# LaurenYTaylor/jsrl-CORL

Hardware: AMD Instinct MI355X
Metric: IQL gradient-steps/sec at batch=256 (D4RL obs/act dims) (higher is better)
Workload: dtype f32; 1 GPU; IQL step on synthetic buffer (obs=17, act=6, 1000000 rows), batch=256 per GPU; global_batch=256, parallelism=single, prepare_rehearsal_steps=1111

## Files before the change

jsrl-corl_amd/csrc/iqlhip.hip:

```cpp
#include "iqlhip_kernels.h"
#include "iqlhip_lb_kernels.h"
#include "iqlhip_owned.h"

#include <dlfcn.h>

#include <time.h>

#include <algorithm>
#include <cstdarg>
#include <cstdio>
#include <cstdlib>
#include <cstring>
#include <memory>
#include <string>
#include <type_traits>
#include <vector>

#define GRAPH_STEPS IQLHIP_GRAPH_STEPS
static const int kChunkSizes[] = {GRAPH_STEPS, 16, 4, 2, 1};

static thread_local std::string g_err;

static int fail(int code, const char* fmt, ...) {
  char buf[512];
// ... 21 lines not shown
  static err_t dev_fill(void* p, int byte, size_t n) { return hipMemset(p, byte, n); }
  static err_t dev_free(void* p) { return hipFree(p); }
  static err_t pin_alloc(void** p, size_t n) { return hipHostMalloc(p, n, hipHostMallocDefault); }
  static err_t pin_free(void* p) { return hipHostFree(p); }
  static err_t event_create(event_t* e, unsigned flags) { return hipEventCreateWithFlags(e, flags); }
  static err_t event_destroy(event_t e) { return hipEventDestroy(e); }
};
using Owned = OwnedT<HipApi>;
extern "C" int64_t iqlhip_debug_live_buffers(void) { return Owned::live().load(std::memory_order_relaxed); }
template <class F> static int all_or_nothing(Owned& own, F&& allocate) {
  const size_t mark = own.mark();
  const int rc = allocate();
  if (rc) own.rollback(mark);
  return rc;
}

template <class F> static auto with_bools(F&& f) { return f(); }
template <class F, class... Bs> static auto with_bools(F&& f, bool b, Bs... rest) {
  if (!b) return with_bools([&](auto... t) { return f(std::false_type{}, t...); }, rest...);
  return with_bools([&](auto... t) { return f(std::true_type{}, t...); }, rest...);
}
static auto fwd_one_kernel(bool bf, bool dma) {
  return with_bools([](auto BF, auto DMA) { return &iql_fwd_kernel<BF.value, DMA.value, false, true>; }, bf, dma);
}
static auto fwd_kernel(bool bf, bool dma, bool multi) {
  return with_bools([](auto MU, auto BF, auto DMA) { return &iql_fwd_kernel<BF.value, DMA.value, MU.value>; }, multi, bf, dma);
}
static auto bwd_kernel(bool bf, bool full, bool multi) {
  return with_bools([](auto MU, auto BF, auto FU) { return &iql_bwd_kernel<BF.value, FU.value, MU.value>; }, multi, bf, full);
}
using BwdRwFn = void (*)(const float*, const float*, const float*, const float*, const float*, unsigned, unsigned, unsigned,
                         unsigned, StepParams, const float*, float*);
static BwdRwFn bwd_rw_kernel(bool full, bool multi);
static auto bwd_rows_kernel(bool csplit) {
  return with_bools([](auto CS) { return &iql_bwd_rows_kernel<CS.value>; }, csplit);
}
template <class Sel> static int set_max_lds(int n_flags, size_t lds, Sel sel) {
  for (unsigned m = 0; m < (1u << n_flags); ++m)
    HIPCHK(hipFuncSetAttribute((const void*)sel(m), hipFuncAttributeMaxDynamicSharedMemorySize, (int)lds));
  return IQLHIP_OK;
}

static inline double now_us() {
  timespec ts;
  clock_gettime(CLOCK_MONOTONIC, &ts);
  return ts.tv_sec * 1e6 + ts.tv_nsec * 1e-3;
}
static const bool g_trace = getenv("IQLHIP_TRACE") != nullptr;

static int check_host_indices(const int64_t* idx_host, int64_t n, int64_t n_rows) {
  for (int64_t i = 0; i < n; ++i)
    if (idx_host[i] < 0 || idx_host[i] >= n_rows)
      return fail(IQLHIP_EINDEX, "index %lld is out of bounds for dimension 0 with size %lld", (long long)idx_host[i], (long long)n_rows);
  return IQLHIP_OK;
}

struct DevGuard {
  int prev = -1;
  bool switched = false;
  explicit DevGuard(int dev) {
    if (hipGetDevice(&prev) == hipSuccess && prev != dev) switched = (hipSetDevice(dev) == hipSuccess);
  }
  ~DevGuard() { if (switched) (void)hipSetDevice(prev); }
};

struct PrioSrc { unsigned* stamp = nullptr; unsigned* flags = nullptr; unsigned long long* delta = nullptr; int sh0 = 0;
// ... 72 lines not shown
  unsigned long long act_drop_seed = 0, act_drop_calls = 0;
  int precision = 0;
  __bf16* wsh = nullptr;
  __bf16* tsh = nullptr;
  float* loss_ring = nullptr;
  int ring_cap = 0;
  iqlhip_step_scalars* sched_cur = nullptr;
  iqlhip_step_scalars* sched_call = nullptr;
  iqlhip_step_scalars* sched_pin[4] = {nullptr, nullptr, nullptr, nullptr};
  unsigned long long* sched_ack = nullptr;
  unsigned long long sched_want[4] = {0, 0, 0, 0};
  unsigned long long call_seq = 0;
  unsigned* setup_arrivals = nullptr;
  bool fwd_lds_set[N_CHUNK_KINDS] = {false, false, false, false, false};
  float* is_buf = nullptr;
  char* prio_buf = nullptr;
  char* prep_save = nullptr;
  hipStream_t sched_stream[4] = {nullptr, nullptr, nullptr, nullptr};
  int sched_slot = 0;
  unsigned long long* hdr = nullptr;
  unsigned long long* stamps = nullptr;
  int k_max = 0;
  int n_chunk_max = 0, n_rt_max = 0;
  size_t lds_fwd = 0, lds_fwd_solo = 0, lds_bwd = 0;
  int n_cus = 256;
  int w0_lds_k = 0;
  int bwd_donate_pct = -1;
  int bwd_spb_force = -1;
  int fwd_spb_force = -1;
  float* pi_t = nullptr;
  __bf16* dh1g = nullptr;
  float* slab_x = nullptr;
  __bf16* wimg = nullptr;
  int lb_enabled = 1;
  int lb_nbb_force = -1, lb_cpb_force = -1, lb_nbi_force = -1;
  bool lb_pi_spread = true;
  bool lb_csplit = true;
  int lb_bwd_part = 0;
  size_t lds_bwd_lb = 0;
  hipStream_t cap_stream = nullptr;
  struct CachedGraph { GraphKey key; hipGraph_t graph; hipGraphExec_t exec; unsigned long long stamp; hipStream_t last;
                       IdleWork* work;
                       hipGraphNode_t setup_node;  };
  struct { bool valid = false; const float* rows = nullptr; int64_t ld = 0, size = 0; int32_t B = 0; uint64_t seed = 0;
           uint64_t next_offset = 0; float drop_p = 0.f; uint64_t drop_seed = 0, drop_step = 0;
           uint64_t wt_gen = 0;
           int cont_class = 0;
           uint64_t wt_ver = 0;
           const void* owner = nullptr;
         } cont;
  std::vector<CachedGraph> graphs;
  unsigned long long graph_clock = 0;
  int xch_mode = IQLHIP_XCH_NONE;
  int rank = 0, world = 1;
  float* xflat = nullptr;
  void* nccl_comm = nullptr;
  char* xblk = nullptr;
  size_t xblk_bytes = 0, xflat_off[2] = {0, 0};
  size_t xslabb_off[2] = {0, 0}, xloss_off[2] = {0, 0};
  long long xslab_b_off[4] = {0, 0, 0, 0};
  char* peer_blk[IQLHIP_MAX_WORLD] = {nullptr, nullptr, nullptr, nullptr, nullptr, nullptr, nullptr, nullptr};
  bool p2p_attached = false;
  unsigned long long* xstatus = nullptr;
  unsigned long long* xstatus_host = nullptr;
  unsigned long long xstep = 0;
  unsigned long long xtimeout_ticks = 500000000ull;
// ... 112 lines not shown
    sb += (size_t)c->n_rt_max * ((size_t)HID * c->L.net[n].k_in + HID);
  }
  HIPCHK(dalloc(&c->sc.slab_b, sb));
  HIPCHK(dalloc(&c->sc.loss_parts, 2 * 4 * 64));
  HIPCHK(dalloc(&c->pi_t, (size_t)MB * 65));
  HIPCHK(dalloc(&c->sc.losses, 4));
  HIPCHK(dalloc(&c->flat_tmp, (size_t)c->L.n_params + 4));
  c->k_max = 1024;
  c->ring_cap = c->k_max;
  HIPCHK(own.pin(&c->loss_ring, (size_t)c->ring_cap * 4 * sizeof(float), true));
  HIPCHK(own.dev(&c->sched_cur, (size_t)GRAPH_STEPS * sizeof(iqlhip_step_scalars)));
  HIPCHK(own.dev(&c->sched_call, (size_t)c->k_max * sizeof(iqlhip_step_scalars)));
  for (int i = 0; i < 4; ++i) HIPCHK(own.pin(&c->sched_pin[i], (size_t)c->k_max * sizeof(iqlhip_step_scalars)));
  HIPCHK(own.pin(&c->sched_ack, 8 * sizeof(unsigned long long), true));
  HIPCHK(own.dev(&c->setup_arrivals, 64, 0));
  HIPCHK(own.dev(&c->hdr, HDR_WORDS * sizeof(unsigned long long), 0));
  HIPCHK(own.dev(&c->xstatus, 2 * sizeof(unsigned long long), 0));
  HIPCHK(own.pin(&c->xstatus_host, 2 * sizeof(unsigned long long), true));
  HIPCHK(dalloc(&c->xflat, (size_t)up(c->L.n_params + 4, 64)));
  HIPCHK(hipStreamCreateWithFlags(&c->cap_stream, hipStreamNonBlocking));
#ifdef IQL_STAMPS
  HIPCHK(own.dev(&c->stamps, 4096 * 16 * sizeof(unsigned long long), 0));
#endif
  const int kq = dims->state_dim + dims->action_dim;
  const int ks_ = dims->state_dim;
  const size_t fwd_fixed = (size_t)(RT_ROWS * H0_LD + RT_ROWS * T64_LD + RT_ROWS * (int)c->row_ld +
                                    (((A + 15) & ~15) * W2_LD + 32) + 512 + 16) * sizeof(float);
  auto fits = [&](int k) { return fwd_fixed + (size_t)HID * k * sizeof(float) + 4096 <= (size_t)160 * 1024 - 1024; };
  int w0_lds_k = 0;
  if (kq <= W0_DMA_MAX_K && fits(kq)) w0_lds_k = kq;
  else if (ks_ <= W0_DMA_MAX_K && fits(ks_)) w0_lds_k = ks_;
  if (const char* ov = getenv("IQLHIP_W0_LDS_K")) w0_lds_k = std::min(w0_lds_k, atoi(ov));
  c->w0_lds_k = w0_lds_k;
  if (const char* ov = getenv("IQLHIP_BWD_DONATE_PCT")) c->bwd_donate_pct = std::max(0, std::min(100, atoi(ov)));
  if (const char* ov = getenv("IQLHIP_BWD_SPB_L2")) c->bwd_spb_force = std::max(0, std::min(2, atoi(ov)));
  if (const char* ov = getenv("IQLHIP_FWD_SPB_L2")) c->fwd_spb_force = std::max(0, std::min(2, atoi(ov)));
  if (const char* ov = getenv("IQLHIP_LB")) c->lb_enabled = atoi(ov) != 0;
  if (const char* ov = getenv("IQLHIP_LB_NBB")) c->lb_nbb_force = std::max(2, atoi(ov));
  if (const char* ov = getenv("IQLHIP_LB_CSPLIT")) c->lb_csplit = atoi(ov) != 0;
  if (const char* ov = getenv("IQLHIP_LB_PI_SPREAD")) c->lb_pi_spread = atoi(ov) != 0;
  if (const char* ov = getenv("IQLHIP_LB_CPB")) c->lb_cpb_force = std::max(1, atoi(ov));
  if (const char* ov = getenv("IQLHIP_LB_NBI")) c->lb_nbi_force = std::max(2, atoi(ov));
  c->lds_fwd = fwd_fixed + (size_t)HID * w0_lds_k * sizeof(float) + (w0_lds_k > W0_LDS_MAX_K ? 4096 : 0);
  c->lds_fwd_solo = std::max(c->lds_fwd, (size_t)(81 * 1024));
  {
    int ncu = 0;
    if (hipDeviceGetAttribute(&ncu, hipDeviceAttributeMultiprocessorCount, c->device) == hipSuccess && ncu > 0) c->n_cus = ncu;
  }
  const int dyld = ((A + 15) & ~15) + 4;
  const size_t lds_a = (size_t)(4 * 32 * T64_LD + 2 * CHUNK_ROWS * dyld + 32 * 32 + 64 + CHUNK_ROWS) * sizeof(float);
  const size_t lds_b = (size_t)(RT_ROWS * H0_LD + 4 * 32 * T64_LD + RT_ROWS * T64_LD + RT_ROWS * 36 + 4 +
                                RT_ROWS * XR_LD_MAX) * sizeof(float);
  c->lds_bwd = std::max(lds_a, lds_b);
  c->lds_bwd_lb = (size_t)(3 * 32 * H0B_LD + 32 * LB_DYLD) * 2 + 32 * 4 + (size_t)(2 * 4 * 32 + 16) * 4;
  int rc = set_max_lds(3, c->lds_fwd_solo, [](unsigned m) { return fwd_kernel(m & 1, m & 2, m & 4); });
  if (!rc) rc = set_max_lds(2, c->lds_fwd_solo, [](unsigned m) { return fwd_one_kernel(m & 1, m & 2); });
  if (!rc) rc = set_max_lds(3, c->lds_bwd, [](unsigned m) { return bwd_kernel(m & 1, m & 2, m & 4); });
  if (!rc) rc = set_max_lds(1, c->lds_bwd_lb, [](unsigned m) { return bwd_rows_kernel(m & 1); });
  if (!rc) rc = set_max_lds(2, c->lds_bwd, [](unsigned m) { return bwd_rw_kernel(m & 1, m & 2); });
  c->fwd_lds_set[(int)ChunkKind::Plain] = !rc;
  return rc;
}

extern "C" int iqlhip_create(const iqlhip_dims* dims, const iqlhip_hyper* hyper, int device, iqlhip_ctx** out) {
  int rc = check_dims(dims);
  if (rc) return rc;
  if (!hyper || !out) return fail(IQLHIP_EINVAL, "hyper/out is NULL");
  int ndev = 0;
  HIPCHK(hipGetDeviceCount(&ndev));
  if (device < 0 || device >= ndev) return fail(IQLHIP_EHIP, "device %d not available (%d visible)", device, ndev);
  DevGuard guard(device);
  iqlhip_ctx* c = new iqlhip_ctx();
  rc = create_impl(c, dims, hyper, device);
  if (rc) {
    const std::string msg = g_err;
    iqlhip_destroy(c);
    g_err = msg;
    return rc;
  }
  *out = c;
  return IQLHIP_OK;
}

static void free_graph(iqlhip_ctx::CachedGraph& g) {
  if (g.exec) (void)hipGraphExecDestroy(g.exec);
  if (g.graph) (void)hipGraphDestroy(g.graph);
  if (g.work) (void)hipFree(g.work);
}
static void drop_graph(iqlhip_ctx* c) {
  for (auto& g : c->graphs) {
    if (g.last) (void)hipStreamSynchronize(g.last);
    free_graph(g);
// ... 296 lines not shown
  u.n_loss = u.n_chunk;
  u.slab_x = nullptr;
  u.n_x = 0;
  if (use_lb(c, rows)) {
    const LbGeom gm = lb_geom(c, rows);
    u.n_chunk = gm.n_cg;
    u.slab_x = c->slab_x;
    u.n_x = gm.nbb;
    u.loss_parts = c->sc.loss_parts + 256;
    u.n_loss = 1;
  }
  u.batch_rows = rows;
  u.sched = nullptr;
  u.sched_idx = 0;
  u.ring_hdr = nullptr;
  u.adv_hdr = nullptr; u.adv_k = 0; u.adv_rows = 0;
  u.done_flag = nullptr; u.done_val = 0;
  u.wsh = (c->precision == 1) ? c->wsh : nullptr;
  u.tsh = (c->precision == 1) ? c->tsh : nullptr;
  u.wimg = (c->precision == 1 && use_lb(c, rows)) ? c->wimg : nullptr;
  if (getenv("IQLHIP_LB_NOIMG")) u.wimg = nullptr;
  u.n_peer = 0;
  u.peer_direct = 0;
  for (int r = 0; r < IQLHIP_MAX_WORLD; ++r) { u.peer_flat[r] = nullptr; u.peer_slab_b[r] = nullptr; u.peer_loss[r] = nullptr; }
  return u;
}

static size_t fwd_lds(const iqlhip_ctx* c, int n_blocks) { return (n_blocks <= c->n_cus) ? c->lds_fwd_solo : c->lds_fwd; }

static const void* fwd_kernel_of(ChunkKind kind, bool bf, bool dma, bool multi);
static void launch_fwd_grid(const iqlhip_ctx* c, const StepParams& p, int nb, hipStream_t st, ChunkKind kind = ChunkKind::Plain) {
  const bool dma = c->w0_lds_k > W0_LDS_MAX_K;
  const bool bf = c->precision == 1, multi = (p.spb_l2 & 3) > 0;
  const void* kernel = (p.only_inst >= 0) ? (const void*)fwd_one_kernel(bf, dma) : fwd_kernel_of(kind, bf, dma, multi);
  void* args[] = {const_cast<StepParams*>(&p)};
  (void)hipLaunchKernel(kernel, dim3(nb), dim3(256), args, fwd_lds(c, nb), st);
}
static int ensure_fwd_lds(iqlhip_ctx* c, ChunkKind kind) {
  if (c->fwd_lds_set[(int)kind]) return IQLHIP_OK;
  DevGuard guard(c->device);
  if (int rc = set_max_lds(3, c->lds_fwd_solo, [kind](unsigned m) { return fwd_kernel_of(kind, m & 1, m & 2, m & 4); })) return rc;
  c->fwd_lds_set[(int)kind] = true;
  return IQLHIP_OK;
}

static int fwd_spb_l2(const iqlhip_ctx* c, int n_rt) {
  if (c->fwd_spb_force >= 0) return c->fwd_spb_force;
  if (8 * n_rt * NSPLIT <= c->n_cus) return 0;
  if (8 * n_rt * 2 <= c->n_cus) return 1;
  return 2;
}
static int fwd_blocks(int n_rt, int l2) { return (l2 == 2) ? 8 * 2 * ((n_rt + 1) / 2) : 8 * n_rt * (NSPLIT >> l2); }
static void launch_fwd(const iqlhip_ctx* c, const StepParams& p_in, hipStream_t st, ChunkKind kind = ChunkKind::Plain) {
  StepParams p = p_in;
  if (p.only_inst < 0 && use_lb(c, p.rows)) {
    const LbArgs a = lb_args(c, p.rows);
    const int kq = c->dims.state_dim + c->dims.action_dim;
    const dim3 grid(8 * a.nbi);
    const bool spread = a.n_rt > 2 * a.nbi && c->lb_pi_spread;
    if (spread) {
      if (kq <= 32) hipLaunchKernelGGL((iql_fwd_lb_kernel<1, true>), grid, dim3(256), 0, st, p, a);
      else if (kq <= 64) hipLaunchKernelGGL((iql_fwd_lb_kernel<2, true>), grid, dim3(256), 0, st, p, a);
      else hipLaunchKernelGGL((iql_fwd_lb_kernel<3, true>), grid, dim3(256), 0, st, p, a);
    } else {
      if (kq <= 32) hipLaunchKernelGGL((iql_fwd_lb_kernel<1, false>), grid, dim3(256), 0, st, p, a);
      else if (kq <= 64) hipLaunchKernelGGL((iql_fwd_lb_kernel<2, false>), grid, dim3(256), 0, st, p, a);
      else hipLaunchKernelGGL((iql_fwd_lb_kernel<3, false>), grid, dim3(256), 0, st, p, a);
// ... 3737 lines not shown
                                        float alpha, float eps, void* stream) {
  if (!t || (m > 0 && (!idx_dev || !td_dev))) return fail(IQLHIP_EINVAL, "NULL argument");
  if (!t->local) return fail(IQLHIP_EINVAL, "the table is not updatable (iqlhip_weights_build_updatable)");
  if (m < 0) return fail(IQLHIP_EINVAL, "m = %lld entries", (long long)m);
  if (bound < 0 || bound > t->n) return fail(IQLHIP_EINVAL, "bound = %lld outside [0, %lld]", (long long)bound, (long long)t->n);
  if ((((uintptr_t)idx_dev) & 7) || (((uintptr_t)td_dev) & 7)) return fail(IQLHIP_EINVAL, "indices and TD errors must be 8-byte aligned");
  if (int rc = prio_exponents_check(alpha, eps)) return rc;
  DevGuard guard(t->device);
  hipStream_t st = (hipStream_t)stream;
  const WUpd u{t->tab, t->stamp, t->flags, (unsigned)t->n, t->levels, t->sh0, t->sat_bits};
  const PrioArgs a{nullptr, alpha, eps};
  for (int64_t j0 = 0; j0 < m; j0 += WT_UPDATE_SLICE) {
    const unsigned k = (unsigned)std::min<int64_t>(WT_UPDATE_SLICE, m - j0);
    launch_update_td(u, (const long long*)idx_dev + j0, td_dev + 2 * j0, k, (long long)bound, t->delta, a, st, t->q_max);
  }
  HIPCHK(hipGetLastError());
  ++t->version;
  return IQLHIP_OK;
}

static auto fwd_prio_kernel(bool dma, bool multi) {
  return with_bools([](auto MU, auto DMA) { return &iql_fwd_prio_kernel<DMA.value, MU.value>; }, multi, dma);
}
static const void* fwd_kernel_of(ChunkKind kind, bool bf, bool dma, bool multi) {
  switch (kind) {
    case ChunkKind::Plain: return (const void*)fwd_kernel(bf, dma, multi);
    case ChunkKind::Mixed: return (const void*)fwd_mixed_kernel(bf, dma, multi);
    case ChunkKind::Weighted: return (const void*)fwd_weighted_kernel(bf, dma, multi);
    case ChunkKind::WeightedIs: return (const void*)fwd_weighted_is_kernel(dma, multi);
    case ChunkKind::Prio: return (const void*)fwd_prio_kernel(dma, multi);
  }
  return nullptr;
}
static void launch_prio_update(const iqlhip_ctx* c, const ChunkSrc& src, int B, int k, hipStream_t st) {
  const WUpd u{const_cast<unsigned long long*>(src.wt.tab), src.up.stamp, src.up.flags, src.wt.n, (int)src.wt.levels, src.up.sh0,
               src.up.sat_bits};
  const PrioArgs a{prio_words(c), 0.f, 0.f};
  launch_update_td(u, prio_idx(c, k & 1), prio_td(c), (unsigned)B, (long long)src.wt.n, src.up.delta, a, st, src.up.q_max);
}
static int prio_setup(iqlhip_ctx* c, const iqlhip_weights* table, int32_t B, float alpha, float eps) {
  if (!table->local) return fail(IQLHIP_EINVAL, "the table is not updatable (iqlhip_weights_build_updatable)");
  if (int rc = prio_exponents_check(alpha, eps)) return rc;
  if (B > WT_UPDATE_SLICE) return fail(IQLHIP_EUNSUPPORTED, "prioritised calls take batches of at most %d rows", WT_UPDATE_SLICE);
  DevGuard guard(c->device);
  if (!c->prio_buf) HIPCHK(c->own.dev(&c->prio_buf, 24 * (size_t)c->dims.max_batch + 4 * sizeof(float), 0));
  return ensure_fwd_lds(c, ChunkKind::Prio);
}
static ChunkCall prio_call(const iqlhip_weights* t, float is_beta, float alpha, float eps, unsigned live) {
  ChunkCall call = weighted_call(t, ChunkKind::Prio, is_beta);
  call.src.up = PrioSrc{t->stamp, t->flags, t->delta, t->sh0, t->sat_bits, t->q_max};
  call.alpha = alpha; call.eps = eps; call.live = live;
  return call;
}
extern "C" int iqlhip_train_steps_prioritized_prepare(iqlhip_ctx* c, const float* rows_dev, int64_t ld, int32_t B,
                                                      float inv_batch, void* stream, iqlhip_weights* table) {
  int rc = check_weighted_args(c, rows_dev, ld, table ? table->n : 0, B, table);
  if (!rc) rc = weighted_is_setup(c, 0.f);
  if (!rc) rc = prio_setup(c, table, B, 1.f, 1.f);
  if (rc) return rc;
  return train_steps_prepare(c, rows_dev, ld, B, inv_batch, stream, prio_call(table, 0.f, 1.f, 1.f, 0u));
}
extern "C" int iqlhip_train_steps_prioritized(iqlhip_ctx* c, const float* rows_dev, int64_t ld, int64_t size, int32_t B,
                                              const iqlhip_step_scalars* sc, int32_t K, uint64_t seed, uint64_t stream_offset,
                                              int32_t flags, void* stream, iqlhip_weights* table, float is_beta, float alpha,
                                              float eps) {
  if (!sc) return fail(IQLHIP_EINVAL, "NULL argument");
// ... 644 lines not shown
```

jsrl-corl_amd/csrc/iqlhip_fwd_body.inc:

```
  RT_ENTRY();
  const int bid = blockIdx.x;
  const int fx = bid & 7, fh = fx >> 2, fr = bid >> 3;
  constexpr unsigned FWD_PAIR_A = 0x6541u, FWD_PAIR_B = 0x7320u;
  const int inst = ONE ? p.only_inst : (int)((((fr & 1) ? FWD_PAIR_B : FWD_PAIR_A) >> (4 * (fx & 3))) & 7u);
  if (inst >= 7) {
    if (p.g_work) idle_block_work<MIXED_IDLE>(p.g_work, (fr >> 1) * 2 + fh, (int)(gridDim.x >> 3));
    return;
  }
  const int spb_l2 = MULTI ? (p.spb_l2 & 3) : 0;
  const int spb = 1 << spb_l2;
  int ns, rt;
  if (ONE) {
    ns = bid & (NSPLIT - 1);
    rt = bid >> 2;
  } else if (spb_l2 == 0) {
    ns = 2 * ((fr >> 1) & 1) + fh;
    rt = fr >> 2;
    if (ROW_EXIT && rt * RT_ROWS >= p.rows) return;
  } else if (spb_l2 == 1) {
    ns = 2 * fh;
    rt = fr >> 1;
    if (ROW_EXIT && rt * RT_ROWS >= p.rows) return;
  } else {
    ns = 0;
    rt = 2 * (fr >> 1) + fh;
    if (rt * RT_ROWS >= p.rows) return;
  }
  const int row0 = rt * RT_ROWS;
  const int tid = threadIdx.x, lane = tid & 63, wave = tid >> 6;
  const int l15 = lane & 15, g = lane >> 4;

  const NetPtrs np = p.inst[inst];
  const int xoff = p.xoff[inst];
  const int slot = p.slot[inst];
  const int k0 = np.k0;
  const int k0p = (k0 + 3) & ~3;
  const int D = np.d;
  const int ld = p.ld;
  const int B = p.rows;
  const int w0k = p.w0_lds_k;
  const float* xb = p.xb;
  float* h0g = p.sc.h0;
  float* h1g = p.sc.h1;
  float* headsg = p.sc.heads;
  const int MB = p.sc.max_batch;
  const int Aact = p.A;
  PIN_P(np.w0); PIN_P(np.b0); PIN_P(np.w1); PIN_P(np.b1); PIN_P(np.w2); PIN_P(np.b2);
  PIN_S(k0); PIN_S(D); PIN_S(xoff); PIN_S(slot); PIN_S(ld); PIN_S(B); PIN_S(MB); PIN_S(Aact);
  PIN_P(xb); PIN_P(h0g); PIN_P(h1g); PIN_P(headsg); PIN_S(w0k);
  const bool w0_lds = W0DMA ? (k0 <= w0k) : (k0 <= min(w0k, W0_LDS_MAX_K));
  const bool w0_dma = W0DMA && w0_lds && (k0 > W0_LDS_MAX_K);

  extern __shared__ __attribute__((aligned(16))) float smem[];
  float* H0s = smem;
  float* H1s = H0s + RT_ROWS * H0_LD;
  float* Xr = H1s + RT_ROWS * T64_LD;
  float* W2s = Xr + RT_ROWS * ld;
  const int w2s_words = ((Aact + 15) & ~15) * W2_LD + 32;
  unsigned* Mk = (unsigned*)(W2s + w2s_words);
  float* W0s = W2s + w2s_words + 512;

  STAMP_BASE(p, 0);
  STAMP(p, 0);
  const int n_x = RT_ROWS * ld / 4;
  const int x_last = B * ld / 4 - 1;
  f32x4 xr[XR_MAX_F4];
  xr_load(xr, xb, row0 * ld / 4, n_x, x_last);
  f32x4 w2pre[2];
#pragma unroll
  for (int q = 0; q < 2; ++q) {
    const int e = min(tid + 256 * q, D * 16 - 1);
    w2pre[q] = *(const f32x4*)(np.w2 + (unsigned)((e >> 4) * HID + ns * 64 + 4 * (e & 15)));
  }
  const float b2v = np.b2[min(tid, D - 1)];
  f32x4 bias0[4];
#pragma unroll
  for (int ct = 0; ct < 4; ++ct) bias0[ct] = *(const f32x4*)(np.b0 + (unsigned)(wave * 64 + ct * 16 + 4 * g));
  f32x4 bias1 = *(const f32x4*)(np.b1 + (unsigned)(ns * 64 + wave * 16 + 4 * g));
  const bool drop = (inst == 6) && (p.drop_bits != nullptr);
  unsigned mk0 = 0xFFFFFFFFu, mk1 = 0xFFFFFFFFu;
  if (drop) {
    const int mrow = min(row0 + (tid >> 3), B - 1);
    mk0 = p.drop_bits[mrow * 8 + (tid & 7)];
    mk1 = p.drop_bits[(MB + mrow) * 8 + (tid & 7)];
  }
  const int n_w0v = 64 * k0;
  f32x4 w0v[16];
  if (w0_dma) {
    const int nj = (n_w0v + 255) >> 8;
    for (int j = 0; j < nj; ++j)
      lds_dma16(np.w0 + 4 * min(tid + 256 * j, n_w0v - 1), W0s + 4 * (256 * j + 64 * wave));
  } else if (w0_lds) {
#pragma unroll
    for (int j = 0; j < 8; ++j) w0v[j] = *(const f32x4*)(np.w0 + 4u * (unsigned)min(tid + 256 * j, n_w0v - 1));
    if (k0 > 32) {
#pragma unroll
      for (int j = 8; j < 16; ++j) w0v[j] = *(const f32x4*)(np.w0 + 4u * (unsigned)min(tid + 256 * j, n_w0v - 1));
    }
  }
  int n1 = ns * 64 + wave * 16 + l15;
  f32x4 bw[BF16 ? 1 : 16];
  bf16x8 bwb[BF16 ? 8 : 1];
  __bf16* H0b = (__bf16*)H0s;

  xr_store(xr, Xr, n_x);
  const int Dp = (D + 15) & ~15;
#pragma unroll
  for (int q = 0; q < 2; ++q) {
    const int e = tid + 256 * q;
    if (e < Dp * 16) *(f32x4*)(W2s + (e >> 4) * W2_LD + 4 * (e & 15)) = (e < D * 16) ? w2pre[q] : (f32x4){0.f, 0.f, 0.f, 0.f};
  }
  if (tid < D) W2s[Dp * W2_LD + tid] = b2v;
  Mk[tid] = mk0;
  Mk[256 + tid] = mk1;
  if (w0_lds && !w0_dma) {
#pragma unroll
    for (int j = 0; j < 8; ++j) {
      const int f = tid + 256 * j;
      if (f < n_w0v) *(f32x4*)(W0s + 4 * f) = w0v[j];
    }
    if (k0 > 32) {
#pragma unroll
      for (int j = 8; j < 16; ++j) {
        const int f = tid + 256 * j;
        if (f < n_w0v) *(f32x4*)(W0s + 4 * f) = w0v[j];
      }
    }
  }
  __syncthreads();
  const bool bw_in_l0 = !BF16 && w0_lds;
#define BW_LOAD(ks_) bw[ks_] = *(const f32x4*)(np.w1 + (unsigned)(n1 * HID + 16 * (ks_) + 4 * g))
#define BWB_AT(unit_, j_) (*(const bf16x8*)((const __bf16*)np.w1 + (unsigned)((unit_) * HID + 32 * (j_) + 8 * g)))
  if constexpr (BF16) {
#pragma unroll
    for (int j = 0; j < 8; ++j) bwb[j] = BWB_AT(n1, j);
  } else if (!bw_in_l0) {
#pragma unroll
    for (int ks = 0; ks < 16; ++ks) BW_LOAD(ks);
  }
  STAMP(p, 1);

  {
    f32x4 acc[2][4];
#pragma unroll
    for (int i = 0; i < 2; ++i)
#pragma unroll
      for (int j = 0; j < 4; ++j) acc[i][j] = (f32x4){0.f, 0.f, 0.f, 0.f};
    const int nks = k0p >> 2;
    const float* x0 = Xr + l15 * ld + xoff;
    const float* x1 = Xr + (16 + l15) * ld + xoff;
    float bcur[4], bnxt[4], acur[2], anxt[2];
    if (w0_lds && nks <= 8) {
      const float* wl[4];
#pragma unroll
      for (int ct = 0; ct < 4; ++ct) wl[ct] = W0s + (wave * 64 + ct * 16 + l15) * k0;
      float bq[8][4], aq[8][2];
#pragma unroll
      for (int ks = 0; ks < 8; ++ks) {
        const int kk = 4 * ks + g;
        const int kc = min(kk, k0 - 1);
#pragma unroll
        for (int ct = 0; ct < 4; ++ct) bq[ks][ct] = wl[ct][kc];
        const float xa = x0[kc], xb_ = x1[kc];
        aq[ks][0] = (kk < k0) ? xa : 0.f;
        aq[ks][1] = (kk < k0) ? xb_ : 0.f;
      }
#pragma unroll
      for (int ks = 0; ks < 8; ++ks) {
        asm volatile("" : "+v"(aq[ks][0]), "+v"(aq[ks][1]));
      }
      STAMP(p, 5);
      if constexpr (BF16) {
        l0_chunk_bf16(acc, bq, aq);
      } else {
// ... 92 lines not shown
          acc[0][ct] = MFMA16(bcur[ct], a0, acc[0][ct]);
          acc[1][ct] = MFMA16(bcur[ct], a1, acc[1][ct]);
        }
#pragma unroll
        for (int ct = 0; ct < 4; ++ct) bcur[ct] = bnxt[ct];
      }
    }
#pragma unroll
    for (int ct = 0; ct < 4; ++ct) {
#pragma unroll
      for (int rtile = 0; rtile < 2; ++rtile) {
        f32x4 h;
#pragma unroll
        for (int reg = 0; reg < 4; ++reg) h[reg] = fmaxf(acc[rtile][ct][reg] + bias0[ct][reg], 0.f);
        if (drop) {
          const unsigned bits = Mk[(rtile * 16 + l15) * 8 + wave * 2 + (ct >> 1)] >> ((ct & 1) * 16 + 4 * g);
#pragma unroll
          for (int reg = 0; reg < 4; ++reg) h[reg] = ((bits >> reg) & 1u) ? h[reg] * p.drop_scale : 0.f;
        }
        if constexpr (BF16) {
          bf16x4 hb_;
#pragma unroll
          for (int reg = 0; reg < 4; ++reg) hb_[reg] = (__bf16)h[reg];
          *(bf16x4*)(H0b + (rtile * 16 + l15) * H0B_LD + wave * 64 + ct * 16 + 4 * g) = hb_;
        } else {
          *(f32x4*)(H0s + (rtile * 16 + l15) * H0_LD + wave * 64 + ct * 16 + 4 * g) = h;
        }
      }
    }
  }
  STAMP(p, 7);
  __syncthreads();
  STAMP(p, 2);

  for (int it = 0;; ++it) {
  const bool more = MULTI && (it + 1 < spb);
  f32x4 bias1n = bias1;
  if (more) {
#pragma unroll
    for (int q = 0; q < 2; ++q) {
      const int e = min(tid + 256 * q, D * 16 - 1);
      w2pre[q] = *(const f32x4*)(np.w2 + (unsigned)((e >> 4) * HID + (ns + 1) * 64 + 4 * (e & 15)));
    }
    bias1n = *(const f32x4*)(np.b1 + (unsigned)((ns + 1) * 64 + wave * 16 + 4 * g));
  }
  if (slot >= 0) {
    const int rl = tid >> 3;
    const int row = row0 + rl;
    if (row < B) {
#pragma unroll
      for (int j = 0; j < 2; ++j) {
        const int col = ns * 64 + 4 * ((tid & 7) + 8 * j);
        if constexpr (BF16)
          *(bf16x4*)((__bf16*)h0g + (unsigned)((slot * MB + row) * HID + col)) = *(const bf16x4*)(H0b + rl * H0B_LD + col);
        else
          *(f32x4*)(h0g + (unsigned)((slot * MB + row) * HID + col)) = *(const f32x4*)(H0s + rl * H0_LD + col);
      }
    }
  }

  if (it == 0) STAMP(p, 8);
  {
    f32x4 acc0 = (f32x4){0.f, 0.f, 0.f, 0.f}, acc1 = acc0;
    if constexpr (BF16) {
      bf16x8 b0[8], b1[8];
#pragma unroll
      for (int j = 0; j < 8; ++j) {
        b0[j] = *(const bf16x8*)(H0b + l15 * H0B_LD + 32 * j + 8 * g);
        b1[j] = *(const bf16x8*)(H0b + (16 + l15) * H0B_LD + 32 * j + 8 * g);
      }
#pragma unroll
      for (int j = 0; j < 8; ++j) {
        acc0 = MFMA_BF16(bwb[j], b0[j], acc0);
        acc1 = MFMA_BF16(bwb[j], b1[j], acc1);
        if ((j & 1) && more) {
          bwb[j - 1] = BWB_AT(n1 + 64, j - 1);
          bwb[j] = BWB_AT(n1 + 64, j);
        }
      }
    } else {
#pragma unroll
      for (int ks = 0; ks < 16; ++ks) {
        const f32x4 a0 = *(const f32x4*)(H0s + l15 * H0_LD + 16 * ks + 4 * g);
        const f32x4 a1 = *(const f32x4*)(H0s + (16 + l15) * H0_LD + 16 * ks + 4 * g);
#pragma unroll
        for (int t = 0; t < 4; ++t) {
          acc0 = MFMA16(bw[ks][t], a0[t], acc0);
          acc1 = MFMA16(bw[ks][t], a1[t], acc1);
        }
        if ((ks & 3) == 3 && more) {
#pragma unroll
          for (int k2 = ks - 3; k2 <= ks; ++k2)
            bw[k2] = *(const f32x4*)(np.w1 + (unsigned)((n1 + 64) * HID + 16 * k2 + 4 * g));
        }
      }
    }
    if (it == 0) STAMP(p, 9);
// ... 91 lines not shown
```

jsrl-corl_amd/csrc/iqlhip_kernels.h:

```cpp
#pragma once
#include <hip/hip_runtime.h>
#include <stdint.h>
#include "iqlhip.h"

typedef float f32x4 __attribute__((ext_vector_type(4)));
typedef float f32x2 __attribute__((ext_vector_type(2)));
typedef float f32x4u __attribute__((ext_vector_type(4), aligned(4)));

#define HID 256
#define RT_ROWS 32
#define CHUNK_ROWS 256
#define H0_LD 260
#define H0B_LD 264
#define T64_LD 68
#define NSPLIT 4
#define HEAD_LD 24
#define W0_LDS_MAX_K 64
#define W0_DMA_MAX_K 96
#define W2_LD 68

#define MFMA16(a, b, c) __builtin_amdgcn_mfma_f32_16x16x4f32((a), (b), (c), 0, 0, 0)

typedef __bf16 bf16x8 __attribute__((ext_vector_type(8)));
#define MFMA_BF16(a, b, c) __builtin_amdgcn_mfma_f32_16x16x32_bf16((a), (b), (c), 0, 0, 0)
// ... 300 lines not shown
                      size, blk * 256 + (int)threadIdx.x, nblk * 256);
  if (blk == nblk - 1 && threadIdx.x < sizeof(iqlhip_step_scalars) / sizeof(float))
    ((float*)w.sched_dst)[threadIdx.x] = ((const float*)(w.sched_call + base + (unsigned long long)w.k))[threadIdx.x];
  if (w.drop_dst)
    dropmask_words(w.drop_dst, w.drop_words, w.drop_thresh, dseed, dstep + (unsigned long long)(w.k + 1),
                   (nblk - 1 - blk) * 256 + (int)threadIdx.x, nblk * 256);
}

__device__ __forceinline__ void l0_chunk_bf16(f32x4 (&acc)[2][4], const float (&bq)[8][4], const float (&aq)[8][2]) {
  bf16x8 B[2];
#pragma unroll
  for (int r = 0; r < 2; ++r) {
    float t8[8];
#pragma unroll
    for (int e = 0; e < 8; ++e) t8[e] = aq[e][r];
    B[r] = pack8s(t8);
  }
#pragma unroll
  for (int ct = 0; ct < 4; ++ct) {
    float t8[8];
#pragma unroll
    for (int e = 0; e < 8; ++e) t8[e] = bq[e][ct];
    const bf16x8 A = pack8s(t8);
    acc[0][ct] = MFMA_BF16(A, B[0], acc[0][ct]);
    acc[1][ct] = MFMA_BF16(A, B[1], acc[1][ct]);
  }
}

template <bool BF16, bool W0DMA, bool MULTI, bool ONE = false>
__global__ __launch_bounds__(256) __attribute__((amdgpu_waves_per_eu(2))) void iql_fwd_kernel(StepParams p) {
  constexpr bool ROW_EXIT = false;
  constexpr bool MIXED_IDLE = false;
#include "iqlhip_fwd_body.inc"
}

struct RowIn {
  f32x4 h[6];
  float r, d;
};

__device__ __forceinline__ void row_issue(const StepParams& p, int row, RowIn& in) {
  const float* hb = p.sc.heads;
  const unsigned o = (unsigned)row * (unsigned)HEAD_LD;
#pragma unroll
  for (int i = 0; i < 6; ++i) in.h[i] = *(const f32x4*)(hb + (o + 4u * i));
  const float* xb = p.xb;
  const unsigned ox = (unsigned)row * (unsigned)p.ld + (unsigned)(2 * p.S + p.A);
  in.r = xb[ox];
  in.d = xb[ox + 1u];
}

__device__ __forceinline__ void row_issue_hot(const float* heads, const float* xb, int ld, int S, int A, int row, RowIn& in) {
  const unsigned o = (unsigned)row * (unsigned)HEAD_LD;
#pragma unroll
  for (int i = 0; i < 6; ++i) in.h[i] = *(const f32x4*)(heads + (o + 4u * i));
  const unsigned ox = (unsigned)row * (unsigned)ld + (unsigned)(2 * S + A);
  in.r = xb[ox];
  in.d = xb[ox + 1u];
}

__device__ __forceinline__ float sum4(const f32x4 v) { return ((v[0] + v[1]) + v[2]) + v[3]; }

__device__ __forceinline__ float tanh_via_exp(float x) {
  const float e = __builtin_amdgcn_exp2f(x * 2.885390081777927f);
  return 1.f - 2.f * __builtin_amdgcn_rcpf(e + 1.f);
}
// ... 1299 lines not shown
```

Measured before the change: 52310 steps/s.

## Add pipelined forward kernel interleaving layer-0 and layer-1 MFMA stages

Result: slower. 51700 steps/s (-1.2%).

```diff
diff --git a/jsrl-corl_amd/csrc/iqlhip.hip b/jsrl-corl_amd/csrc/iqlhip.hip
--- a/jsrl-corl_amd/csrc/iqlhip.hip
+++ b/jsrl-corl_amd/csrc/iqlhip.hip
@@ -77,6 +77,7 @@
 using BwdRwFn = void (*)(const float*, const float*, const float*, const float*, const float*, unsigned, unsigned, unsigned,
                          unsigned, StepParams, const float*, float*);
 static BwdRwFn bwd_rw_kernel(bool full, bool multi);
+static const void* fwd_pipe_kernel();
 static auto bwd_rows_kernel(bool csplit) {
   return with_bools([](auto CS) { return &iql_bwd_rows_kernel<CS.value>; }, csplit);
 }
@@ -215,6 +216,8 @@
   __bf16* dh1g = nullptr;
   float* slab_x = nullptr;
   __bf16* wimg = nullptr;
+  int fwd_pipe = 1;
+  bool fwd_pipe_ok = false;
   int lb_enabled = 1;
   int lb_nbb_force = -1, lb_cpb_force = -1, lb_nbi_force = -1;
   bool lb_pi_spread = true;
@@ -393,6 +396,8 @@
   else if (ks_ <= W0_DMA_MAX_K && fits(ks_)) w0_lds_k = ks_;
   if (const char* ov = getenv("IQLHIP_W0_LDS_K")) w0_lds_k = std::min(w0_lds_k, atoi(ov));
   c->w0_lds_k = w0_lds_k;
+  c->fwd_pipe_ok = kq <= 32 && w0_lds_k >= kq;
+  if (const char* ov = getenv("IQLHIP_FWD_PIPE")) c->fwd_pipe = atoi(ov) != 0;
   if (const char* ov = getenv("IQLHIP_BWD_DONATE_PCT")) c->bwd_donate_pct = std::max(0, std::min(100, atoi(ov)));
   if (const char* ov = getenv("IQLHIP_BWD_SPB_L2")) c->bwd_spb_force = std::max(0, std::min(2, atoi(ov)));
   if (const char* ov = getenv("IQLHIP_FWD_SPB_L2")) c->fwd_spb_force = std::max(0, std::min(2, atoi(ov)));
@@ -419,6 +424,7 @@
   if (!rc) rc = set_max_lds(3, c->lds_bwd, [](unsigned m) { return bwd_kernel(m & 1, m & 2, m & 4); });
   if (!rc) rc = set_max_lds(1, c->lds_bwd_lb, [](unsigned m) { return bwd_rows_kernel(m & 1); });
   if (!rc) rc = set_max_lds(2, c->lds_bwd, [](unsigned m) { return bwd_rw_kernel(m & 1, m & 2); });
+  if (!rc) rc = set_max_lds(0, c->lds_fwd_solo, [](unsigned) { return fwd_pipe_kernel(); });
   c->fwd_lds_set[(int)ChunkKind::Plain] = !rc;
   return rc;
 }
@@ -781,7 +787,10 @@
 static void launch_fwd_grid(const iqlhip_ctx* c, const StepParams& p, int nb, hipStream_t st, ChunkKind kind = ChunkKind::Plain) {
   const bool dma = c->w0_lds_k > W0_LDS_MAX_K;
   const bool bf = c->precision == 1, multi = (p.spb_l2 & 3) > 0;
-  const void* kernel = (p.only_inst >= 0) ? (const void*)fwd_one_kernel(bf, dma) : fwd_kernel_of(kind, bf, dma, multi);
+  const bool pipe = c->fwd_pipe && c->fwd_pipe_ok && kind == ChunkKind::Plain && !bf && !dma && !multi && p.only_inst < 0;
+  const void* kernel = (p.only_inst >= 0) ? (const void*)fwd_one_kernel(bf, dma)
+                       : pipe             ? fwd_pipe_kernel()
+                                          : fwd_kernel_of(kind, bf, dma, multi);
   void* args[] = {const_cast<StepParams*>(&p)};
   (void)hipLaunchKernel(kernel, dim3(nb), dim3(256), args, fwd_lds(c, nb), st);
 }
@@ -4585,6 +4594,7 @@
   }
   return nullptr;
 }
+static const void* fwd_pipe_kernel() { return (const void*)&iql_fwd_pipe_kernel<4>; }
 static void launch_prio_update(const iqlhip_ctx* c, const ChunkSrc& src, int B, int k, hipStream_t st) {
   const WUpd u{const_cast<unsigned long long*>(src.wt.tab), src.up.stamp, src.up.flags, src.wt.n, (int)src.wt.levels, src.up.sh0,
                src.up.sat_bits};
diff --git a/jsrl-corl_amd/csrc/iqlhip_fwd_body.inc b/jsrl-corl_amd/csrc/iqlhip_fwd_body.inc
--- a/jsrl-corl_amd/csrc/iqlhip_fwd_body.inc
+++ b/jsrl-corl_amd/csrc/iqlhip_fwd_body.inc
@@ -1,4 +1,9 @@
   RT_ENTRY();
+#ifdef IQL_FWD_PIPE_BODY
+  constexpr bool PIPE = true;
+#else
+  constexpr bool PIPE = false;
+#endif
   const int bid = blockIdx.x;
   const int fx = bid & 7, fh = fx >> 2, fr = bid >> 3;
   constexpr unsigned FWD_PAIR_A = 0x6541u, FWD_PAIR_B = 0x7320u;
@@ -48,7 +53,7 @@
   PIN_P(np.w0); PIN_P(np.b0); PIN_P(np.w1); PIN_P(np.b1); PIN_P(np.w2); PIN_P(np.b2);
   PIN_S(k0); PIN_S(D); PIN_S(xoff); PIN_S(slot); PIN_S(ld); PIN_S(B); PIN_S(MB); PIN_S(Aact);
   PIN_P(xb); PIN_P(h0g); PIN_P(h1g); PIN_P(headsg); PIN_S(w0k);
-  const bool w0_lds = W0DMA ? (k0 <= w0k) : (k0 <= min(w0k, W0_LDS_MAX_K));
+  const bool w0_lds = PIPE ? true : W0DMA ? (k0 <= w0k) : (k0 <= min(w0k, W0_LDS_MAX_K));
   const bool w0_dma = W0DMA && w0_lds && (k0 > W0_LDS_MAX_K);
 
   extern __shared__ __attribute__((aligned(16))) float smem[];
@@ -75,7 +80,8 @@
   const float b2v = np.b2[min(tid, D - 1)];
   f32x4 bias0[4];
 #pragma unroll
-  for (int ct = 0; ct < 4; ++ct) bias0[ct] = *(const f32x4*)(np.b0 + (unsigned)(wave * 64 + ct * 16 + 4 * g));
+  for (int ct = 0; ct < 4; ++ct)
+    bias0[ct] = *(const f32x4*)(np.b0 + (unsigned)((PIPE ? ct * 64 + wave * 16 : wave * 64 + ct * 16) + 4 * g));
   f32x4 bias1 = *(const f32x4*)(np.b1 + (unsigned)(ns * 64 + wave * 16 + 4 * g));
   const bool drop = (inst == 6) && (p.drop_bits != nullptr);
   unsigned mk0 = 0xFFFFFFFFu, mk1 = 0xFFFFFFFFu;
@@ -93,7 +99,7 @@
   } else if (w0_lds) {
 #pragma unroll
     for (int j = 0; j < 8; ++j) w0v[j] = *(const f32x4*)(np.w0 + 4u * (unsigned)min(tid + 256 * j, n_w0v - 1));
-    if (k0 > 32) {
+    if (!PIPE && k0 > 32) {
 #pragma unroll
       for (int j = 8; j < 16; ++j) w0v[j] = *(const f32x4*)(np.w0 + 4u * (unsigned)min(tid + 256 * j, n_w0v - 1));
     }
@@ -119,7 +125,7 @@
       const int f = tid + 256 * j;
       if (f < n_w0v) *(f32x4*)(W0s + 4 * f) = w0v[j];
     }
-    if (k0 > 32) {
+    if (!PIPE && k0 > 32) {
 #pragma unroll
       for (int j = 8; j < 16; ++j) {
         const int f = tid + 256 * j;
@@ -140,6 +146,126 @@
   }
   STAMP(p, 1);
 
+  f32x4 pacc0 = (f32x4){0.f, 0.f, 0.f, 0.f}, pacc1 = pacc0;
+  if constexpr (PIPE) {
+#define SB() __builtin_amdgcn_sched_barrier(0)
+    const int nks = k0p >> 2;
+    const float* x0 = Xr + l15 * ld + xoff;
+    const float* x1 = Xr + (16 + l15) * ld + xoff;
+    const float* wl = W0s + (wave * 16 + l15) * k0;
+    float aq[8][2], bq[4][8];
+    int kcs[8];
+#pragma unroll
+    for (int ks = 0; ks < 8; ++ks) {
+      const int kk = 4 * ks + g;
+      kcs[ks] = min(kk, k0 - 1);
+      const float xa = x0[kcs[ks]], xb_ = x1[kcs[ks]];
+      aq[ks][0] = (kk < k0) ? xa : 0.f;
+      aq[ks][1] = (kk < k0) ? xb_ : 0.f;
+    }
+#pragma unroll
+    for (int q = 0; q < 4; ++q)
+#pragma unroll
+      for (int ks = 0; ks < 8; ++ks) bq[q][ks] = wl[64 * q * k0 + kcs[ks]];
+#pragma unroll
+    for (int ks = 0; ks < 8; ++ks) asm volatile("" : "+v"(aq[ks][0]), "+v"(aq[ks][1]));
+    SB();
+#pragma unroll
+    for (int k2 = 0; k2 < 4; ++k2) BW_LOAD(k2);
+    SB();
+    STAMP(p, 5);
+    f32x4 acc[4][2];
+#pragma unroll
+    for (int q = 0; q < 4; ++q) acc[q][0] = acc[q][1] = (f32x4){0.f, 0.f, 0.f, 0.f};
+    auto l0 = [&](const int q) {
+#pragma unroll
+      for (int ks = 0; ks < 8; ++ks) {
+        if (ks < nks) {
+          acc[q][0] = MFMA16(bq[q][ks], aq[ks][0], acc[q][0]);
+          acc[q][1] = MFMA16(bq[q][ks], aq[ks][1], acc[q][1]);
+        }
+      }
+    };
+    auto epi = [&](const int q) {
+#pragma unroll
+      for (int rtile = 0; rtile < 2; ++rtile) {
+        f32x4 h;
+#pragma unroll
+        for (int reg = 0; reg < 4; ++reg) h[reg] = fmaxf(acc[q][rtile][reg] + bias0[q][reg], 0.f);
+        if (drop) {
+          const unsigned bits = Mk[(rtile * 16 + l15) * 8 + 2 * q + (wave >> 1)] >> ((wave & 1) * 16 + 4 * g);
+#pragma unroll
+          for (int reg = 0; reg < 4; ++reg) h[reg] = ((bits >> reg) & 1u) ? h[reg] * p.drop_scale : 0.f;
+        }
+        *(f32x4*)(H0s + (rtile * 16 + l15) * H0_LD + 64 * q + 16 * wave + 4 * g) = h;
+      }
+    };
+    auto h0_save = [&]() {
+      if (slot >= 0) {
+        const int rl = tid >> 3;
+        const int row = row0 + rl;
+        if (row < B) {
+#pragma unroll
+          for (int j = 0; j < 2; ++j) {
+            const int col = ns * 64 + 4 * ((tid & 7) + 8 * j);
+            *(f32x4*)(h0g + (unsigned)((slot * MB + row) * HID + col)) = *(const f32x4*)(H0s + rl * H0_LD + col);
+          }
+        }
+      }
+    };
+    l0(0);
+    SB();
+#pragma unroll
+    for (int k2 = 4; k2 < 8; ++k2) BW_LOAD(k2);
+    SB();
+    l0(1);
+    SB();
+#pragma unroll
+    for (int k2 = 8; k2 < 12; ++k2) BW_LOAD(k2);
+    SB();
+    epi(0);
+    SB();
+#pragma unroll
+    for (int q = 0; q < 4; ++q) {
+      __syncthreads();
+      SB();
+      f32x4 a0[4], a1[4];
+#pragma unroll
+      for (int t4 = 0; t4 < 4; ++t4) {
+        a0[t4] = *(const f32x4*)(H0s + l15 * H0_LD + 16 * (4 * q + t4) + 4 * g);
+        a1[t4] = *(const f32x4*)(H0s + (16 + l15) * H0_LD + 16 * (4 * q + t4) + 4 * g);
+      }
+      if (q == 0) {
+#pragma unroll
+        for (int k2 = 12; k2 < 16; ++k2) BW_LOAD(k2);
+      }
+      if (q == ns && q < 3) h0_save();
+      SB();
+      if (q + 2 < 4) {
+        l0(q + 2);
+        SB();
+      }
+      if (q == 1) STAMP(p, 6);
+      if (q == 0) STAMP(p, 2);
+#pragma unroll
+      for (int t4 = 0; t4 < 4; ++t4) {
+#pragma unroll
+        for (int t = 0; t < 4; ++t) {
+          pacc0 = MFMA16(bw[4 * q + t4][t], a0[t4][t], pacc0);
+          pacc1 = MFMA16(bw[4 * q + t4][t], a1[t4][t], pacc1);
+        }
+        if (t4 == 0 && q + 1 < 4) {
+          SB();
+          epi(q + 1);
+          SB();
+          if (q == 2) STAMP(p, 7);
+        }
+      }
+      SB();
+      if (q == 3 && ns == 3) h0_save();
+    }
+#undef SB
+  } else {
   {
     f32x4 acc[2][4];
 #pragma unroll
@@ -298,6 +424,7 @@
   STAMP(p, 7);
   __syncthreads();
   STAMP(p, 2);
+  }
 
   for (int it = 0;; ++it) {
   const bool more = MULTI && (it + 1 < spb);
@@ -310,7 +437,7 @@
     }
     bias1n = *(const f32x4*)(np.b1 + (unsigned)((ns + 1) * 64 + wave * 16 + 4 * g));
   }
-  if (slot >= 0) {
+  if (!PIPE && slot >= 0) {
     const int rl = tid >> 3;
     const int row = row0 + rl;
     if (row < B) {
@@ -328,7 +455,10 @@
   if (it == 0) STAMP(p, 8);
   {
     f32x4 acc0 = (f32x4){0.f, 0.f, 0.f, 0.f}, acc1 = acc0;
-    if constexpr (BF16) {
+    if constexpr (PIPE) {
+      acc0 = pacc0;
+      acc1 = pacc1;
+    } else if constexpr (BF16) {
       bf16x8 b0[8], b1[8];
 #pragma unroll
       for (int j = 0; j < 8; ++j) {
diff --git a/jsrl-corl_amd/csrc/iqlhip_kernels.h b/jsrl-corl_amd/csrc/iqlhip_kernels.h
--- a/jsrl-corl_amd/csrc/iqlhip_kernels.h
+++ b/jsrl-corl_amd/csrc/iqlhip_kernels.h
@@ -356,6 +356,17 @@
   constexpr bool ROW_EXIT = false;
   constexpr bool MIXED_IDLE = false;
 #include "iqlhip_fwd_body.inc"
+}
+
+template <int NSTAGE>
+__global__ __launch_bounds__(256) __attribute__((amdgpu_waves_per_eu(2))) void iql_fwd_pipe_kernel(StepParams p) {
+  static_assert(NSTAGE == 4, "four stages of 64 columns: one per k-step group of layer 1 and per column slice");
+  constexpr bool BF16 = false, W0DMA = false, MULTI = false, ONE = false;
+  constexpr bool ROW_EXIT = false;
+  constexpr bool MIXED_IDLE = false;
+#define IQL_FWD_PIPE_BODY 1
+#include "iqlhip_fwd_body.inc"
+#undef IQL_FWD_PIPE_BODY
 }
 
 struct RowIn {
```
